# romi/plant-3d-vision

Measured on AMD Instinct MI355X. Metric: Mvoxels*views/sec space-carve, 512^3 x 72 views per MI355X, higher is better.
Workload: dtype f32

## Files before the change

plant-3d-vision_amd/csrc/sc_bricks.h:

```cpp

template <bool ALL_SAFE = false>
__device__ __forceinline__ void two_views(const ViewDesc &da, const ViewDesc &db, bool two, float x, float y,
                                          const float (&z)[4], unsigned long long (&alive)[4], unsigned long long (&kept)[4]) {
    const float aax = da.R[0] * x + da.R[1] * y, aay = da.R[3] * x + da.R[4] * y, aaz = da.R[6] * x + da.R[7] * y;
    const float bax = db.R[0] * x + db.R[1] * y, bay = db.R[3] * x + db.R[4] * y, baz = db.R[6] * x + db.R[7] * y;
    const uint32_t rowa = (uint32_t)da.strip, rowb = (uint32_t)db.strip;
    unsigned long long oka[4], okb[4];
    uint32_t wa[4], wb[4];
    int sha[4], shb[4];
#pragma unroll
    for (int e = 0; e < 4; ++e) {
        int v;
        bool ok = project<ALL_SAFE>(aax, aay, aaz, z[e], da, sha[e], v, oka[e]);
        wa[e] = load_mask_at(da.mask, ok ? mask_byte_offset(sha[e], v, rowa) : 0u);
        ok = project<ALL_SAFE>(bax, bay, baz, z[e], db, shb[e], v, okb[e]);
        wb[e] = load_mask_at(db.mask, ok ? mask_byte_offset(shb[e], v, rowb) : 0u);
    }
    const unsigned long long second = two ? ~0ull : 0ull;
#pragma unroll
    for (int e = 0; e < 4; ++e) {
        unsigned long long fg = __ballot(__builtin_amdgcn_ubfe(wa[e], (uint32_t)sha[e], 1u) != 0u);
        unsigned long long seen = oka[e] & alive[e];
        alive[e] &= ~(seen & ~fg);
        kept[e] |= seen & fg;
        fg = __ballot(__builtin_amdgcn_ubfe(wb[e], (uint32_t)shb[e], 1u) != 0u);
        seen = okb[e] & alive[e] & second;
        alive[e] &= ~(seen & ~fg);
        kept[e] |= seen & fg;
    }
}

__device__ __forceinline__ void labels_behind(int32_t (&lab)[4], const unsigned long long (&alive)[4],
                                              const unsigned long long (&kept)[4]) {
#pragma unroll
    for (int e = 0; e < 4; ++e) {
        const int32_t up = lab[e] == 0 ? 1 : lab[e];
        const int32_t live = __builtin_amdgcn_inverse_ballot_w64(kept[e]) ? up : lab[e];
        lab[e] = __builtin_amdgcn_inverse_ballot_w64(alive[e]) ? live : -1;
    }
}

template <bool FRESH, bool ALL_SAFE = false>
__device__ __forceinline__ void brick_voxels(int32_t *__restrict__ labels, const GridDesc &g,
                                             const ViewDesc *__restrict__ views, int nviews,
                                             int32_t init, Append ap, uint32_t il, uint32_t j,
                                             uint32_t k0, uint32_t lb, uint32_t lane, uint32_t unit = 0,
                                             int nextra = 0) {
    const bool inside = j < g.ny && k0 < g.nz;
    const int nvalid = inside ? (int)min(4u, g.nz - k0) : 0;
    const uint64_t elem = ((uint64_t)il * g.ny + j) * g.nzp + k0;
    int32_t *p = labels + elem;
    int32_t lab[4], was[4];
#pragma unroll
    for (int e = 0; e < 4; ++e) lab[e] = -1;
    if (FRESH) {
#pragma unroll
        for (int e = 0; e < 4; ++e)
            if (e < nvalid) lab[e] = init;
    } else if (inside) {
        int4 q = *reinterpret_cast<const int4 *>(p);
        lab[0] = q.x; lab[1] = q.y; lab[2] = q.z; lab[3] = q.w;
#pragma unroll
        for (int e = 0; e < 4; ++e)
            if (e >= nvalid) lab[e] = -1;
    }
    unsigned long long alive[4], kept[4];
#pragma unroll
    for (int e = 0; e < 4; ++e) {
        was[e] = lab[e];
        alive[e] = __ballot(lab[e] != -1);
        kept[e] = 0;
    }
    const float x = g.ox + (float)(int)(il * g.istride + g.i0) * g.vs;
    const float y = g.oy + (float)(int)j * g.vs;
    float z[4];
#pragma unroll
    for (int e = 0; e < 4; ++e) z[e] = g.oz + (float)(int)(k0 + e) * g.vs;

    for (int vi = 0; vi < nviews; vi += 2) {
        if ((alive[0] | alive[1] | alive[2] | alive[3]) == 0) break;
        const bool two = vi + 1 < nviews;
        const ViewDesc da = views[vi];
        const ViewDesc db = views[two ? vi + 1 : vi];
        two_views<ALL_SAFE>(da, db, two, x, y, z, alive, kept);
    }
    if (nextra >= 2 && ap.list != nullptr) {
        const uint32_t left = (uint32_t)(__popcll(alive[0]) + __popcll(alive[1]) + __popcll(alive[2]) + __popcll(alive[3]));
        if (left >= 32u && left <= 128u) {
            const ViewDesc da = views[nviews];
            const ViewDesc db = views[nviews + 1];
            two_views<ALL_SAFE>(da, db, true, x, y, z, alive, kept);
        }
    }
    labels_behind(lab, alive, kept);

    const bool changed = FRESH || lab[0] != was[0] || lab[1] != was[1] || lab[2] != was[2] || lab[3] != was[3];
    if (inside && changed) *reinterpret_cast<int4 *>(p) = make_int4(lab[0], lab[1], lab[2], lab[3]);

    if (ap.list != nullptr) {
        ap.sub = (lb * 0x9E3779B1u) >> 24;
        uint32_t total = 0;
#pragma unroll
        for (int e = 0; e < 4; ++e) total += (uint32_t)__popcll(alive[e]);
        bool bulked = false;
        if (ap.bulk != nullptr && total >= ap.bulk_min) {
            uint32_t pos = 0;
            if (lane == 0) pos = atomicAdd(&ap.ctl->count[3][ap.sub].n, 1u);
            pos = __shfl(pos, 0);
            bulked = pos < ap.bulkcap;
            if (bulked && lane == 0)
                ap.bulk[(size_t)ap.sub * ap.bulkcap + pos] = lb * 4u + unit;
        }
        if (total != 0 && !bulked) {
            uint32_t base = 0;
            if (lane == 0) base = atomicAdd(&ap.ctl->count[0][ap.sub].n, total);
            base = __shfl(base, 0);
            if (base + total > ap.subcap) {
                if (lane == 0) ap.ctl->overflow = 1u;
            } else {
                uint32_t *dst = ap.list + (size_t)ap.sub * ap.subcap + base;
                uint32_t rank = 0;
#pragma unroll
                for (int e = 0; e < 4; ++e) rank += lanes_below(alive[e]);
#pragma unroll
                for (int e = 0; e < 4; ++e) {
                    if (__builtin_amdgcn_inverse_ballot_w64(alive[e])) {
                        dst[rank] = (uint32_t)(elem + e) | (lab[e] == 0 ? 0x80000000u : 0u);
                        ++rank;
                    }
                }
            }
        }
    }
}

struct Fill {
    int32_t kept;
    int32_t fresh;
    int32_t init;
};

__device__ __forceinline__ uint32_t strip_flag(const uint8_t *__restrict__ flags, uint32_t strip, uint32_t bricks_z) {
    const uint32_t lane = threadIdx.x & 63;
    return (lane < bricks_z) ? flags[strip * bricks_z + lane] : 0u;
}
__device__ __forceinline__ void store_culled_bricks(int32_t *__restrict__ labels, const GridDesc &g, uint32_t f, uint32_t strip,
                                                    uint32_t bricks_y, uint32_t bricks_z, Fill fill, bool prefilled = false) {
    typedef int v4i __attribute__((ext_vector_type(4)));
    const uint32_t wave = __builtin_amdgcn_readfirstlane(threadIdx.x >> 6), lane = threadIdx.x & 63;
    const uint32_t il = strip / bricks_y, by = strip - il * bricks_y;
    const uint32_t j0 = by * kBrickY + wave * 4, j = j0 + (lane >> 4);
    const unsigned long long culled = prefilled ? 0ull : __ballot(f == 1u), full = __ballot(f == 2u);
    const unsigned long long untouched = fill.fresh ? __ballot(f == 6u) : 0ull;
    if (j >= g.ny) return;
    const uint32_t l16 = lane & 15u;
    const bool tail_ok = (bricks_z - 1u) * kBrickZ + l16 * 4u < g.nz;
    const unsigned long long last = 1ull << (bricks_z - 1u);
    {
        const char *wbase = reinterpret_cast<const char *>(labels) + ((uint64_t)il * g.ny + j0) * g.nzp * 4u;
        const uint32_t voff = (lane >> 4) * g.nzp * 4u + l16 * 16u;
        v4i minus = {-1, -1, -1, -1};
        asm volatile("" : "+v"(minus));
        unsigned long long body = culled & ~last;
        while (body != 0) {
            const uint32_t bz = (uint32_t)__builtin_ctzll(body);
            body &= body - 1;
            asm volatile("global_store_dwordx4 %0, %1, %2 nt" ::"v"(voff), "v"(minus), "s"(wbase + bz * 256u) : "memory");
        }
        if ((culled & last) != 0 && tail_ok)
            asm volatile("global_store_dwordx4 %0, %1, %2 nt" ::"v"(voff), "v"(minus), "s"(wbase + (bricks_z - 1u) * 256u) : "memory");
        asm volatile("s_nop 1" ::"v"(minus));
    }
    unsigned long long rest = full | untouched;
    if (rest == 0) return;
    int32_t *col = labels + ((uint64_t)il * g.ny + j) * g.nzp;
    while (rest != 0) {
        const uint32_t bz = (uint32_t)__builtin_ctzll(rest);
        rest &= rest - 1;
        const bool isfull = (full >> bz) & 1ull;
        const uint32_t k0 = bz * kBrickZ + l16 * 4;
        if (k0 >= g.nz) continue;
        if (!isfull || fill.fresh) {
            const int32_t val = isfull ? fill.kept : fill.init;
            const v4i vv = {val, val, val, val};
            __builtin_nontemporal_store(vv, reinterpret_cast<v4i *>(col + k0));
        } else {
            const uint32_t n = min(4u, g.nz - k0);
            for (uint32_t e = 0; e < n; ++e)
                if (col[k0 + e] == 0) col[k0 + e] = 1;
        }
    }
}

#ifdef SC_TRACE_DENSE
__device__ uint32_t g_dense_trace[8192 * 8];
#endif
constexpr int kConfirmWaves = 8;
struct UnitRoad {
    int32_t *labels;
    int32_t init, fresh;
    uint32_t nbricks;
};

__global__ __launch_bounds__(64 * kConfirmWaves) void brick_confirm_kernel(
    GridDesc g, const ViewDesc *__restrict__ views, int v0, int v1, uint32_t bricks_y, uint32_t bricks_z,
    uint8_t *__restrict__ flags, const uint32_t *__restrict__ cands, uint32_t cand_per, uint32_t *__restrict__ late,
    ListCtl *ctl, uint32_t parity, UnitRoad ur) {
    if (v0 >= v1) return;
    uint32_t ncand[kCandSub], gfirst[kCandSub + 1];
    gfirst[0] = 0;
#pragma unroll
    for (int s = 0; s < kCandSub; ++s) {
        ncand[s] = ctl->ncand[parity][s].n;
        gfirst[s + 1] = gfirst[s] + ((ncand[s] + 63u) >> 6);
    }
    __shared__ unsigned long long s_full[kConfirmWaves], s_seen[kConfirmWaves];
    __shared__ unsigned long long s_road, s_rseen;
    const uint32_t wave = __builtin_amdgcn_readfirstlane(threadIdx.x >> 6), lane = threadIdx.x & 63u;
    const uint32_t per_plane = bricks_y * bricks_z;
    for (uint32_t grp = blockIdx.x; grp < gfirst[kCandSub]; grp += gridDim.x) {
        uint32_t sub = 0, first = 0, n = ncand[0];
#pragma unroll
        for (int s = 1; s < kCandSub; ++s)
            if (grp >= gfirst[s]) { sub = (uint32_t)s; first = gfirst[s]; n = ncand[s]; }
        const uint32_t idx = (grp - first) * 64u + lane;
        const bool isc = idx < n;
        const uint32_t lb = isc ? cands[(size_t)sub * cand_per * 64u + idx] : 0u;
        const uint32_t fl = isc ? flags[lb] : 0u;
        unsigned long long any_seen = __ballot(fl == 3u);
        unsigned long long cand = __ballot(isc);
        const uint32_t il = lb / per_plane;
        const uint32_t rem = lb - il * per_plane;
        const uint32_t by = rem / bricks_z, bz = rem - by * bricks_z;
        const float x = g.ox + (float)(int)(il * g.istride + g.i0) * g.vs;
        for (int base = v0; base < v1 && cand != 0; base += kConfirmWaves) {
            const int vi = base + (int)wave;
            bool keeps = true, sees = false;
            if (vi < v1 && ((cand >> lane) & 1ull)) {
                const ViewDesc d = views[vi];
                const uint32_t v = brick_verdict(d, g, x, (int)(by * kBrickY), (int)(bz * kBrickZ), d.tiles_x);
                keeps = v == 2u || v == 4u;
                sees = v == 2u;
            }
            const unsigned long long mf = __ballot(keeps), ms = __ballot(sees);
            __syncthreads();
            if (lane == 0) { s_full[wave] = mf; s_seen[wave] = ms; }
            __syncthreads();
#pragma unroll
            for (int w = 0; w < kConfirmWaves; ++w) { cand &= s_full[w]; any_seen |= s_seen[w]; }
        }
        const bool road = ur.labels != nullptr && ctl->overflow == 0u;
        if (wave == 0) {
            if (isc) flags[lb] = ((cand >> lane) & 1ull) ? (((any_seen >> lane) & 1ull) ? 2 : 6) : 5;
            const bool failed = isc && !((cand >> lane) & 1ull);
            const unsigned long long m = __ballot(failed);
            if (m != 0) {
                uint32_t pos = 0;
                if (lane == 0) pos = atomicAdd(road ? &ctl->nlate_units : &ctl->nlate, (uint32_t)__popcll(m));
                pos = __shfl(pos, 0);
                const unsigned long long below = (lane == 0) ? 0ull : (~0ull >> (64 - lane));
                const uint32_t at = pos + (uint32_t)__popcll(m & below);
                if (failed) late[road ? ur.nbricks - 1u - at : at] = lb;
            }
            if (lane == 0) { s_road = road ? m : 0ull; s_rseen = any_seen; }
        }
        __syncthreads();
        if (road) {
            const unsigned long long mr = s_road, ms = s_rseen;
            uint32_t nth = 0;
            for (unsigned long long mm = mr; mm != 0; mm &= mm - 1, ++nth) {
                if ((nth & (uint32_t)(kConfirmWaves - 1)) != wave) continue;
                const uint32_t src = (uint32_t)__builtin_ctzll(mm);
                const uint32_t b = __builtin_amdgcn_readlane(lb, src);
                const bool seen = (ms >> src) & 1ull;
                const uint32_t bil = b / per_plane, brem = b - bil * per_plane;
                const uint32_t bby = brem / bricks_z, bbz = brem - bby * bricks_z;
                const uint32_t k0 = bbz * kBrickZ + (lane & 15u) * 4u;
#pragma unroll
                for (uint32_t i = 0; i < 4u; ++i) {
                    const uint32_t j = bby * kBrickY + i * 4u + (lane >> 4);
                    if (j >= g.ny || k0 >= g.nz) continue;
                    int32_t *p = ur.labels + ((uint64_t)bil * g.ny + j) * g.nzp + k0;
                    if (ur.fresh) {
                        const int32_t val = (seen && ur.init == 0) ? 1 : ur.init;
                        *reinterpret_cast<int4 *>(p) = make_int4(val, val, val, val);
                    } else if (seen) {
                        int4 q = *reinterpret_cast<const int4 *>(p);
                        const bool changed = q.x == 0 || q.y == 0 || q.z == 0 || q.w == 0;
                        q.x = q.x == 0 ? 1 : q.x; q.y = q.y == 0 ? 1 : q.y; q.z = q.z == 0 ? 1 : q.z; q.w = q.w == 0 ? 1 : q.w;
                        if (changed) *reinterpret_cast<int4 *>(p) = q;
                    }
                }
            }
        }
        __syncthreads();
    }
}

template <bool FRESH, bool ALL_SAFE = false>
__global__ __launch_bounds__(kBlock) __attribute__((amdgpu_num_sgpr(102))) void carve_brick_kernel(int32_t *__restrict__ labels, GridDesc g,
                                                             const ViewDesc *__restrict__ views,
                                                             int nviews, int32_t init, Append ap,
                                                             uint32_t bricks_y, uint32_t bricks_z,
                                                             const uint8_t *__restrict__ flags,
                                                             const uint32_t *__restrict__ live,
                                                             ListCtl *ctl, uint32_t nwalkers,
                                                             PackJob ride, int pack_rows,
                                                             uint32_t parity, int nverd_arg, uint32_t verd_max_live,
                                                             uint32_t bulk_min_live, int nextra) {
    if (blockIdx.x >= nwalkers) {
        const uint32_t b = blockIdx.x - nwalkers;
        const int rs = pack_rows == 0 ? pack_band_slot(ride, b)
                                      : (pack_rows == 1 ? pack16_slot<1>(ride, b)
                                                        : (pack_rows == 2 ? pack16_slot<2>(ride, b) : (pack_rows == 8 ? pack16_slot<8>(ride, b) : pack16_slot<4>(ride, b))));
        if (rs >= ride.nslots) return;
        const TileRect rc = job_rect(ride, rs + ride.slot0);
        uint32_t packed;
        if (pack_rows == 0) packed = pack_band_block(ride, b, rc);
        else if (pack_rows == 1) packed = pack16_block<1>(ride, b, rc);
        else if (pack_rows == 2) packed = pack16_block<2>(ride, b, rc);
        else if (pack_rows == 8) packed = pack16_block<8>(ride, b, rc);
        else packed = pack16_block<4>(ride, b, rc);
        if (packed != 0u && threadIdx.x == 0) (void)atomicAdd(&ctl->rider_tiles[b & (uint32_t)(kRiderCounters - 1)].n, packed);
        return;
    }
    const uint32_t nlive = ctl->nlive[parity];
    const int nverd = nlive <= verd_max_live ? nverd_arg : 0;
    if (nlive < bulk_min_live) ap.bulk = nullptr;
    const uint32_t lane = threadIdx.x & 63;
    const uint32_t per_plane = bricks_y * bricks_z;
    const uint32_t xcd = blockIdx.x & 7u;
    const uint32_t per_xcd = (nwalkers >> 3) * (kBlock / 64);
    bool first = true;
    uint32_t misses = 0, turn = 0;
#ifdef SC_TRACE_DENSE
    const uint64_t tr0 = wall_clock64();
    uint32_t tr_bricks = 0, tr_units = 0, tr_verd = 0, tr_unit = 0, tr_tick = 0;
#endif
    for (;;) {
#ifdef SC_TRACE_DENSE
        const uint64_t tra = wall_clock64();
// ... 158 lines not shown
```

plant-3d-vision_amd/csrc/sc_engine.h:

```cpp

struct sc_engine {
    int device = 0;
    int mode = SC_MODE_CARVE;
    int64_t nx = 0, ny = 0, nz = 0, i0 = 0, istride = 1, planes = 0, n = 0;
    int64_t nzp = 0;
    int64_t npitch = 0;
    void *dense = nullptr;
    float origin[3] = {0, 0, 0};
    float vs = 1.0f;
    float default_value = 0.0f;
    void *state = nullptr;
    bool fresh = true;

    hipStream_t own_stream = nullptr, stream = nullptr;
    std::thread setup_thread;
    bool setup_pending = false;
    int setup_rc = SC_OK;
    std::string setup_err;
    double setup_ms = 0.0;
    double setup_waited_ms = 0.0;

    std::vector<ViewDesc> pending;
    ViewDesc *views_dev = nullptr;
    ViewDesc *views_pin = nullptr;
// ... 473 lines not shown
    for (int q = 0; q < V; ++q) {
        ViewDesc d;
        fill_desc(e, d, K + 4 * q, R + 9 * q, t + 3 * q,
                  static_cast<uint32_t *>(packed) + (size_t)q * words, H, W, occ + (size_t)q * occ_bytes);
        if (cmask) d.cmask = cmask + (size_t)q * occ_bytes;
        e->pending.push_back(d);
    }
    return SC_OK;
}

int enqueue_tile8(sc_engine *e, int V, const float *K, const float *R, const float *t,
                  const void *raw_dev, int H, int W, int64_t row_stride, int64_t view_stride) {
    int tiles_x = (W + kATileW - 1) / kATileW, tiles_y = (H + kATileH - 1) / kATileH;
    size_t per_view = (size_t)tiles_x * tiles_y * 128;
    if (per_view >= ((size_t)1 << 31) || (size_t)tiles_y * 128 >= ((size_t)1 << 24))
        return fail(SC_ERR_INVALID, "mask too large for the byte gather (%d x %d)", W, H);
    void *tiled = nullptr;
    int rc = arena_alloc(e, per_view * (size_t)V, &tiled);
    if (rc) return rc;
    int fast = (W % 16) == 0 && (row_stride % 16) == 0 && (view_stride % 16) == 0 &&
               (reinterpret_cast<uintptr_t>(raw_dev) % 16) == 0;
    int64_t total = (int64_t)V * H * ((W + 15) / 16);
    int64_t blocks = (total + kBlock - 1) / kBlock;
    if (blocks > 0x7fffffffLL) return fail(SC_ERR_INVALID, "mask batch too large");
    const size_t uni_per_view = (size_t)((W + 31) / 32) * (size_t)((H + 31) / 32);
    uint8_t *uni = nullptr;
    if (fast && e->avg_brick) {
        void *u = nullptr;
        size_t bytes = (uni_per_view * (size_t)V + 3) & ~(size_t)3;
        rc = arena_alloc(e, bytes, &u);
        if (rc) return rc;
        uni = static_cast<uint8_t *>(u);
    }
    LaunchTimer lt{e, SC_KERNEL_PACK};
    rc = lt.begin();
    if (rc) return rc;
    hipLaunchKernelGGL(tile8_kernel, dim3((uint32_t)blocks), dim3(kBlock), 0, e->stream,
                       static_cast<const uint8_t *>(raw_dev), row_stride, view_stride, W, H, V, tiles_x,
                       tiles_y, static_cast<uint8_t *>(tiled), fast);
    if (uni) {
        int64_t ntiles = (int64_t)V * (int64_t)uni_per_view;
        hipLaunchKernelGGL(uniform_tiles_kernel, dim3((uint32_t)((ntiles + 3) / 4)), dim3(kBlock), 0, e->stream,
                           static_cast<const uint8_t *>(tiled), W, H, V, tiles_x, tiles_y, uni);
    }
    HIP_TRY(hipGetLastError());
    rc = lt.end();
    if (rc) return rc;
    for (int q = 0; q < V; ++q) {
        ViewDesc d;
        fill_desc(e, d, K + 4 * q, R + 9 * q, t + 3 * q, static_cast<uint8_t *>(tiled) + (size_t)q * per_view, H, W,
                  uni ? uni + (size_t)q * uni_per_view : nullptr);
        d.tiles_x = tiles_y * 128;
        d.pad = 1;
        e->pending.push_back(d);
    }
    return SC_OK;
}

int enqueue_tilef32(sc_engine *e, int V, const float *K, const float *R, const float *t, const void *raw_dev,
                    int H, int W, int64_t row_stride, int64_t view_stride) {
    const int tiles_x = (W + kFTileW - 1) / kFTileW, tiles_y = (H + kFTileH - 1) / kFTileH;
    const size_t per_view = (size_t)tiles_x * tiles_y * 128;
    if (per_view >= ((size_t)1 << 33) || (size_t)tiles_y * 32 >= ((size_t)1 << 24))
        return fail(SC_ERR_INVALID, "mask too large for the float gather (%d x %d)", W, H);
    void *tiled = nullptr;
    int rc = arena_alloc(e, per_view * (size_t)V, &tiled);
    if (rc) return rc;
    const int fast = (W % 4) == 0 && (row_stride % 16) == 0 && (view_stride % 16) == 0 &&
                     (reinterpret_cast<uintptr_t>(raw_dev) % 16) == 0;
    const int64_t total = (int64_t)V * H * ((W + 3) / 4);
    const int64_t blocks = (total + kBlock - 1) / kBlock;
    if (blocks > 0x7fffffffLL) return fail(SC_ERR_INVALID, "mask batch too large");
    const size_t nreg = (size_t)((W + 31) / 32) * (size_t)((H + 31) / 32);
    const size_t uni_view = ((nreg + 3) & ~(size_t)3) + nreg * 4;
    void *u = nullptr;
    rc = arena_alloc(e, uni_view * (size_t)V, &u);
    if (rc) return rc;
    uint8_t *uni = static_cast<uint8_t *>(u);
    LaunchTimer lt{e, SC_KERNEL_PACK};
    rc = lt.begin();
    if (rc) return rc;
    hipLaunchKernelGGL(tilef_kernel, dim3((uint32_t)blocks), dim3(kBlock), 0, e->stream, static_cast<const float *>(raw_dev),
                       row_stride, view_stride, W, H, V, tiles_x, tiles_y, static_cast<float *>(tiled), fast);
    const int64_t regs = (int64_t)V * (int64_t)nreg;
    hipLaunchKernelGGL(uniform_f32_kernel, dim3((uint32_t)((regs + 3) / 4)), dim3(kBlock), 0, e->stream,
                       static_cast<const float *>(tiled), W, H, V, tiles_x, tiles_y, uni, uni_view);
    HIP_TRY(hipGetLastError());
    rc = lt.end();
    if (rc) return rc;
    for (int q = 0; q < V; ++q) {
        ViewDesc d;
        fill_desc(e, d, K + 4 * q, R + 9 * q, t + 3 * q, static_cast<char *>(tiled) + (size_t)q * per_view, H, W,
                  uni + (size_t)q * uni_view);
        d.tiles_x = tiles_y * 32;
        d.pad = 2;
        e->pending.push_back(d);
    }
    return SC_OK;
}

void order_views(std::vector<ViewDesc> &v, std::vector<uint32_t> *perm = nullptr) {
    size_t n = v.size();
    if (perm) {
        perm->resize(n);
        for (size_t q = 0; q < n; ++q) (*perm)[q] = (uint32_t)q;
    }
    if (n < 3 || n > 4096) return;
    std::vector<float> worst(n, 0.0f);
    std::vector<char> used(n, 0);
    std::vector<ViewDesc> out;
    out.reserve(n);
    size_t cur = 0;
    for (size_t step = 0; step < n; ++step) {
        used[cur] = 1;
        out.push_back(v[cur]);
        if (perm) (*perm)[step] = (uint32_t)cur;
        const float *a = v[cur].R + 6;
        size_t best = n;
        for (size_t q = 0; q < n; ++q) {
            if (used[q]) continue;
            const float *b = v[q].R + 6;
            float c = std::fabs(a[0] * b[0] + a[1] * b[1] + a[2] * b[2]);
            if (c > worst[q]) worst[q] = c;
            if (best == n || worst[q] < worst[best]) best = q;
        }
        cur = best;
    }
    v.swap(out);
}

constexpr int kMinFusedViews = 6;

int ensure_lists(sc_engine *e) {
    if (e->lists && e->list_cap_built == e->list_cap) return SC_OK;
    if (e->lists) {
        HIP_TRY(schost::wait_stream(e->stream));
        (void)hipFree(e->lists);
        e->lists = nullptr;
    }
    uint64_t total = std::max<uint64_t>((uint64_t)e->n / 4 + (uint64_t)e->n / 16, (uint64_t)kSub * 1024);
    e->subcap = (uint32_t)((total + kSub - 1) / kSub);
    if (e->list_cap > 0) e->subcap = (uint32_t)e->list_cap;
    HIP_TRY(sc_dev_malloc(reinterpret_cast<void **>(&e->lists), (size_t)2 * kSub * e->subcap * sizeof(uint32_t)));
    e->list_cap_built = e->list_cap;
    return SC_OK;
}

int ensure_ctl(sc_engine *e) {
    if (e->ctl) return SC_OK;
    size_t nbricks = 0;
    if ((e->nz + kBrickZ - 1) / kBrickZ <= 64)
        nbricks = (size_t)e->planes * (size_t)((e->ny + kBrickY - 1) / kBrickY) * (size_t)((e->nz + kBrickZ - 1) / kBrickZ);
    char *base = nullptr;
    size_t flag_bytes = (nbricks + 15) & ~(size_t)15;
    const uint32_t bulkcap = (uint32_t)((nbricks * 4 * 2 + kSub - 1) / kSub + 64);
    const size_t bulk_words = nbricks ? (size_t)kSub * bulkcap : 0;
    const uint32_t itemcap = bulkcap * 5u;
    uint4 *items = nullptr;
    if (bulk_words) HIP_TRY(sc_dev_malloc(reinterpret_cast<void **>(&items), (size_t)kSub * itemcap * sizeof(uint4)));
    hipError_t he = sc_dev_malloc(reinterpret_cast<void **>(&base),
                              2 * sizeof(ListCtl) + flag_bytes + (3 * nbricks + bulk_words) * sizeof(uint32_t) + 16);
    if (he == hipSuccess) he = hipMemsetAsync(base, 0, 2 * sizeof(ListCtl), e->stream);
    if (he != hipSuccess) {
        if (items) (void)hipFree(items);
        if (base) (void)hipFree(base);
        return fail(he == hipErrorOutOfMemory ? SC_ERR_NOMEM : SC_ERR_DEVICE, "control block allocation failed: %s", hipGetErrorString(he));
    }
    e->bulkcap = bulkcap;
    e->itemcap = itemcap;
    e->items = items;
    e->ctl2[0] = reinterpret_cast<ListCtl *>(base);
    e->ctl2[1] = e->ctl2[0] + 1;
    e->ctl_clean[0] = e->ctl_clean[1] = true;
    e->ctl_idx = 0;
    e->ctl = e->ctl2[0];
    e->flags = reinterpret_cast<uint8_t *>(base + 2 * sizeof(ListCtl));
    e->live = reinterpret_cast<uint32_t *>(base + 2 * sizeof(ListCtl) + flag_bytes);
    e->late = e->live + nbricks;
    e->fill_list = e->late + nbricks;
    e->bulk = bulk_words ? e->fill_list + nbricks : nullptr;
    return SC_OK;
}

int deferred_job(sc_engine *e, PackJob *out) {
    const auto &db = e->deferred;
    size_t words = packed_words(db.H, db.W);
    void *packed = nullptr, *occ_v = nullptr;
    int rc = arena_alloc(e, words * 4 * (size_t)db.V, &packed);
    if (rc) return rc;
    const size_t occ_bytes = (size_t)((db.W + kTile - 1) / kTile) * (size_t)((db.H + kTile - 1) / kTile);
    rc = arena_alloc(e, occ_bytes * (size_t)db.V, &occ_v);
    if (rc) return rc;
    uint32_t *cmask = nullptr;
    if (e->bulk_min > 0 || e->unit_cull) {
        void *cv = nullptr;
        rc = arena_alloc(e, occ_bytes * 4 * (size_t)db.V, &cv);
        if (rc) return rc;
        cmask = static_cast<uint32_t *>(cv);
    }
    for (int q = 0; q < db.V; ++q) {
        e->pending[(size_t)q].mask = static_cast<uint32_t *>(packed) + (size_t)q * words;
        e->pending[(size_t)q].occ = static_cast<uint8_t *>(occ_v) + (size_t)q * occ_bytes;
        if (cmask) e->pending[(size_t)q].cmask = cmask + (size_t)q * occ_bytes;
    }
    *out = make_pack_job(db.raw, db.row_stride, db.view_stride, db.W, db.H, static_cast<uint32_t *>(packed),
                         (int64_t)words, pack_flip(db.dtype), static_cast<uint8_t *>(occ_v), cmask);
    return SC_OK;
}

int materialize_deferred(sc_engine *e) {
    if (!e->deferred.on) return SC_OK;
    PackJob pj;
    int rc = deferred_job(e, &pj);
    if (rc) return rc;
    e->deferred.on = false;
    pj.slot0 = 0;
    pj.nslots = e->deferred.V;
    rc = step_begin(e);
    if (rc) return rc;
    LaunchTimer lt{e, SC_KERNEL_PACK};
    rc = lt.begin();
    if (rc) return rc;
    rc = launch_pack16(e, pj);
    if (rc) return rc;
    return lt.end();
}

int hostbits_reserve(sc_engine *e, size_t bytes, char **out) {
    auto &a = e->hb[e->hb_cur];
    if (a.used == 0 && a.armed) {
        HIP_TRY(schost::wait_event(a.ev));
        a.armed = false;
    }
    if (a.used + bytes > a.cap) {
        const size_t cap = std::max<size_t>({a.used + bytes, a.cap * 2, (size_t)16 << 20});
        char *pin = nullptr, *dev = nullptr;
        HIP_TRY(sc_pin_malloc(reinterpret_cast<void **>(&pin), cap, hipHostMallocDefault));
        hipError_t he = sc_dev_malloc(reinterpret_cast<void **>(&dev), cap);
        if (he != hipSuccess) {
            (void)hipHostFree(pin);
            return fail(he == hipErrorOutOfMemory ? SC_ERR_NOMEM : SC_ERR_DEVICE, "host-mask arena: %s", hipGetErrorString(he));
        }
        if (a.used) memcpy(pin, a.pin, a.used);
        if (a.pin) {
            HIP_TRY(schost::wait_stream(e->stream));
            (void)hipHostFree(a.pin);
            (void)hipFree(a.dev);
        }
        a.pin = pin;
        a.dev = dev;
        a.cap = cap;
        a.armed = false;
    }
    if (!a.ev) HIP_TRY(hipEventCreateWithFlags(&a.ev, hipEventDisableTiming));
    *out = a.pin + a.used;
    a.used += bytes;
    return SC_OK;
}

int hostbits_push_view(sc_engine *e, const float *K, const float *R, const float *t, uint64_t src_off, int H, int W);

int enqueue_hostbits(sc_engine *e, const float *K, const float *R, const float *t, const void *mask, int H, int W,
                     int dtype, int64_t row_stride) {
    const int wpr = (W + kTile - 1) / kTile;
    const size_t bits_bytes = ((size_t)H * wpr * 4 + 255) & ~(size_t)255;
    char *dst = nullptr;
    int rc = hostbits_reserve(e, bits_bytes, &dst);
    if (rc) return rc;
    const uint64_t src_off = (uint64_t)(dst - e->hb[e->hb_cur].pin);
    const int elem = dtype == SC_MASK_I32 ? 4 : 1;
    const uint8_t flip = dtype == SC_MASK_U8_INV ? 255 : dtype == SC_MASK_BOOL_INV ? 1 : 0;
    uint32_t *out = reinterpret_cast<uint32_t *>(dst);
    const bool par = (size_t)H * W >= ((size_t)1 << 18);
    const int band = 64, nparts = par ? (H + band - 1) / band : 1;
    schost::parallel_for(nparts, [&](int part) {
        const int r0 = par ? part * band : 0, r1 = par ? std::min(H, r0 + band) : H;
        schost::pack_rows(mask, row_stride, W, r0, r1, out, wpr, elem, flip);
    });
    return hostbits_push_view(e, K, R, t, src_off, H, W);
}

int hostbits_push_view(sc_engine *e, const float *K, const float *R, const float *t, uint64_t src_off, int H, int W) {
    const int wpr = (W + kTile - 1) / kTile, tiles_y = (H + kTile - 1) / kTile;
    const size_t ntiles = (size_t)wpr * tiles_y;
    void *tiles = nullptr, *occ = nullptr, *cm = nullptr;
    int rc = arena_alloc(e, ntiles * 128, &tiles);
    if (rc) return rc;
    rc = arena_alloc(e, ntiles, &occ);
    if (rc) return rc;
    rc = arena_alloc(e, ntiles * 4, &cm);
    if (rc) return rc;
    BitsRec br;
    memset(&br, 0, sizeof br);
    br.src_off = src_off;
    br.tiles = static_cast<uint32_t *>(tiles);
    br.occ = static_cast<uint8_t *>(occ);
    br.cmask = static_cast<uint32_t *>(cm);
    br.W = W; br.H = H; br.tiles_x = wpr; br.tiles_y = tiles_y;
    e->hp_pending.push_back(br);
    ViewDesc d;
    fill_desc(e, d, K, R, t, tiles, H, W, static_cast<const uint8_t *>(occ));
    d.cmask = static_cast<const uint32_t *>(cm);
    e->pending.push_back(d);
    return SC_OK;
}

int upload_hostbits(sc_engine *e) {
// ... 32 lines not shown
```

plant-3d-vision_amd/csrc/sc_lists.h:

```cpp

struct UnitItems {
    const uint4 *items;
    uint32_t cap;
    const ViewDesc *views;
    uint32_t bricks_y, bricks_z;
};

__device__ __forceinline__ uint32_t list_reserve(ListCounter *counter, uint32_t total, uint32_t cap, uint32_t lane) {
    uint32_t base = 0;
    if (lane == 0) {
        base = atomicAdd(&counter->n, total);
        if (base > cap || total > cap - base) {
            atomicMax(&counter->cut, ~min(base, cap));
            base = 0xffffffffu;
        }
    }
    return __shfl(base, 0);
}

struct UnitSpill {
    const uint32_t *units;
    uint32_t cap, floor;
    uint32_t bricks_y, bricks_z;
};

template <bool FINAL, int P, bool ALL_SAFE = false>
__global__ __launch_bounds__(kBlock) __attribute__((amdgpu_num_sgpr(96))) void carve_list_kernel(int32_t *__restrict__ labels, GridDesc g,
                                                            const ViewDesc *__restrict__ views,
                                                            int nviews,
                                                            const uint32_t *__restrict__ lin,
                                                            uint32_t *__restrict__ lout,
                                                            ListCtl *ctl, int sin, int sout,
                                                            uint32_t subcap, int vgsize, CullStores cs, UnitItems ui,
                                                            UnitSpill us, int nrest) {
    static_assert(P == 2, "two survivors per lane: the instances with one and with four were retired in round 6");
    __shared__ uint32_t pref[kSub + 1];
    const uint32_t tid = threadIdx.x;
    const uint32_t bx = blockIdx.x, gdim = gridDim.x;
    const bool split = cs.flags != nullptr;
    const uint32_t nown = cs.nstrips - cs.first, nvirt = nown + cs.spec;
    const uint32_t nstore = split ? (cs.fill_blocks ? cs.fill_blocks : nvirt) : 0u;
    const uint32_t nbid = gdim - nstore;
    if (split && bx >= nbid) {
        constexpr uint32_t kAhead = 4;
        for (uint32_t t = bx - nbid; t < nvirt; t += nstore * kAhead) {
            uint32_t f[kAhead];
#pragma unroll
            for (uint32_t u = 0; u < kAhead; ++u) {
                const uint32_t tt = t + u * nstore;
                f[u] = tt < nvirt ? strip_flag(cs.flags, tt < nown ? cs.first + tt : tt - nown, cs.bricks_z) : 0u;
            }
#pragma unroll
            for (uint32_t u = 0; u < kAhead; ++u) {
                const uint32_t tt = t + u * nstore;
                if (tt < nvirt)
                    store_culled_bricks(labels, g, f[u], tt < nown ? cs.first + tt : tt - nown, cs.bricks_y, cs.bricks_z,
                                        Fill{cs.kept, cs.fresh, cs.init}, tt >= nown);
            }
        }
        return;
    }
    if (ctl->overflow) return;
    const uint32_t bid = bx;
    constexpr uint32_t CH = 64u * P;
    {
        uint32_t c = (list_count(ctl->count[sin][tid], subcap) + CH - 1u) / CH;
        if (tid == 0) pref[0] = 0;
        pref[tid + 1] = c;
        __syncthreads();
        for (uint32_t off = 1; off < kSub; off <<= 1) {
            uint32_t val = pref[tid + 1];
            uint32_t add = (tid >= off) ? pref[tid + 1 - off] : 0u;
            __syncthreads();
            pref[tid + 1] = val + add;
            __syncthreads();
        }
    }
    const uint32_t chunks = pref[kSub];
    const uint32_t lane = tid & 63u;
    __shared__ uint32_t ipref[kSub + 1];
    const bool with_items = FINAL && ui.items != nullptr;
    uint32_t uchunks = 0;
    constexpr uint32_t kUnitParts = 256u / (64u * P);
    if (!FINAL && us.units != nullptr) {
        const uint32_t c = min(ctl->count[3][tid].n, us.cap);
        if (tid == 0) ipref[0] = 0;
        ipref[tid + 1] = c;
        __syncthreads();
        for (uint32_t off = 1; off < kSub; off <<= 1) {
            const uint32_t val = ipref[tid + 1];
            const uint32_t add = (tid >= off) ? ipref[tid + 1 - off] : 0u;
            __syncthreads();
            ipref[tid + 1] = val + add;
            __syncthreads();
        }
        if (ipref[kSub] < us.floor) uchunks = ipref[kSub] * kUnitParts;
    }
    if (with_items) {
        const uint32_t c = list_count(ctl->count[4][tid], ui.cap);
        if (tid == 0) ipref[0] = 0;
        ipref[tid + 1] = c;
        __syncthreads();
        for (uint32_t off = 1; off < kSub; off <<= 1) {
            const uint32_t val = ipref[tid + 1];
            const uint32_t add = (tid >= off) ? ipref[tid + 1 - off] : 0u;
            __syncthreads();
            ipref[tid + 1] = val + add;
            __syncthreads();
        }
    }
    const uint64_t nworkers = (uint64_t)nbid * (kBlock / 64);
    const uint32_t wave = __builtin_amdgcn_readfirstlane(tid >> 6);
    const uint64_t total = FINAL ? (uint64_t)chunks * (uint32_t)nviews : (uint64_t)chunks + uchunks;
    uint64_t per = 1;
    if (FINAL) {
        per = (total + nworkers - 1) / nworkers;
        const uint64_t r = (uint64_t)max(vgsize, 1);
        per = (per + r - 1) / r * r;
    }
    const uint64_t wid = (uint64_t)bid * (kBlock / 64) + wave;
    uint64_t pos = FINAL ? min(total, wid * per) : wid;
    const uint64_t end = FINAL ? min(total, pos + per) : total;
    while (pos < end) {
        uint32_t c;
        int v0, v1;
        if (FINAL) {
            c = (uint32_t)(pos / (uint32_t)nviews);
            v0 = (int)(pos - (uint64_t)c * (uint32_t)nviews);
            v1 = (int)min((uint64_t)nviews, (uint64_t)v0 + (end - pos));
            pos += (uint64_t)(v1 - v0);
        } else {
            c = (uint32_t)pos;
            v0 = 0;
            v1 = nviews;
            pos += nworkers;
        }
        const bool from_unit = !FINAL && c >= chunks;
        const uint32_t *pf = from_unit ? ipref : pref;
        const uint32_t key = from_unit ? (c - chunks) / kUnitParts : c;
        uint32_t lo = 0, hi = kSub;
        while (hi - lo > 1) {
            uint32_t mid = (lo + hi) >> 1;
            if (pf[mid] <= key) lo = mid; else hi = mid;
        }
        const uint32_t s = lo;
        const uint32_t cnt = list_count(ctl->count[sin][s], subcap);
        uint32_t idx[P];
        unsigned long long alive_m[P], zero_m[P], flip_m[P];
        float x[P], y[P], z[P];
        uint32_t unit = 0, upart = 0;
        if (from_unit) {
            unit = __builtin_amdgcn_readfirstlane(us.units[(size_t)s * us.cap + (key - ipref[s])]);
            upart = (c - chunks) % kUnitParts;
        }
#pragma unroll
        for (int p = 0; p < P; ++p) {
            if (from_unit) {
                const uint32_t v = upart * CH + (uint32_t)p * 64u + lane;
                const uint32_t lb = unit >> 2, per_plane = us.bricks_y * us.bricks_z;
                const uint32_t il = lb / per_plane, rem = lb - il * per_plane;
                const uint32_t by = rem / us.bricks_z, bz = rem - by * us.bricks_z;
                const uint32_t j = by * kBrickY + (v >> 4), k = bz * kBrickZ + (unit & 3u) * 16u + (v & 15u);
                const bool inside = j < g.ny && k < g.nz;
                idx[p] = inside ? (il * g.ny + j) * g.nzp + k : 0u;
                int32_t lab = -1;
                if (inside) lab = labels[idx[p]];
                alive_m[p] = __ballot(lab != -1);
                zero_m[p] = __ballot(lab == 0);
            } else {
                const uint32_t e = (c - pref[s]) * CH + (uint32_t)p * 64u + lane;
                const bool in = e < cnt;
                uint32_t entry = 0;
                if (in) entry = lin[(size_t)s * subcap + e];
                idx[p] = entry & 0x7fffffffu;
                alive_m[p] = __ballot(in);
                zero_m[p] = __ballot((entry >> 31) != 0);
            }
            flip_m[p] = 0;
            const uint32_t col = fdiv(idx[p], g.by_nzp);
            const uint32_t k = idx[p] - col * g.nzp;
            const uint32_t il = fdiv(col, g.by_ny);
            const uint32_t j = col - il * g.ny;
            x[p] = g.ox + (float)(int)(il * g.istride + g.i0) * g.vs;
            y[p] = g.oy + (float)(int)j * g.vs;
            z[p] = g.oz + (float)(int)k * g.vs;
        }
        constexpr int U = 4;
        for (;;) {
        for (int vi = v0; vi < v1; vi += U) {
            unsigned long long any = 0;
#pragma unroll
            for (int p = 0; p < P; ++p) any |= alive_m[p];
            if (any == 0) break;
            unsigned long long okm[U][P];
            uint32_t w[U][P];
            int sh[U][P];
#pragma unroll
            for (int q = 0; q < U; ++q) {
                const ViewDesc d = views[vi + q < v1 ? vi + q : vi];
                asm volatile("" ::"s"(d.Wf), "s"(d.Hf), "s"(d.strip), "s"(d.mask));
                const uint32_t tile_row = (uint32_t)d.strip;
#pragma unroll
                for (int p = 0; p < P; ++p) {
                    int vv;
                    const bool ok = project<ALL_SAFE>(d.R[0] * x[p] + d.R[1] * y[p], d.R[3] * x[p] + d.R[4] * y[p],
                                                      d.R[6] * x[p] + d.R[7] * y[p], z[p], d, sh[q][p], vv, okm[q][p]);
                    w[q][p] = 0;
                    if (ok) w[q][p] = load_mask_at(d.mask, mask_byte_offset(sh[q][p], vv, tile_row));
                }
            }
#pragma unroll
// ... 484 lines not shown
```

Before: 68.02 million.

## Read brick flags as scalar words and batch culled-brick stores per strip piece

The store-only blocks of the carve kernel now load each strip's brick flags as three uniform dwords through the constant address space, replacing one per-lane byte load followed by ballots. Flags are decoded eight bricks at a time with SWAR byte compares. A fully culled 8-brick piece takes a fast path that issues eight back-to-back nontemporal stores with immediate offsets. Flag loads are software-pipelined one batch ahead, and the flag buffer gains 12 bytes of padding so the over-read stays in bounds. The cost is more scalar registers and more complex indexing, and the split into 8-brick pieces adds loop iterations when bricks_z is large.

Measured after the change: 65.21 million. -4.1%, worse.

```diff
diff --git a/plant-3d-vision_amd/csrc/sc_bricks.h b/plant-3d-vision_amd/csrc/sc_bricks.h
--- a/plant-3d-vision_amd/csrc/sc_bricks.h
+++ b/plant-3d-vision_amd/csrc/sc_bricks.h
@@ -140,53 +140,100 @@
     int32_t init;
 };
 
-__device__ __forceinline__ uint32_t strip_flag(const uint8_t *__restrict__ flags, uint32_t strip, uint32_t bricks_z) {
-    const uint32_t lane = threadIdx.x & 63;
-    return (lane < bricks_z) ? flags[strip * bricks_z + lane] : 0u;
-}
-__device__ __forceinline__ void store_culled_bricks(int32_t *__restrict__ labels, const GridDesc &g, uint32_t f, uint32_t strip,
-                                                    uint32_t bricks_y, uint32_t bricks_z, Fill fill, bool prefilled = false) {
+struct StripRaw {
+    uint32_t w[3];
+};
+__device__ __forceinline__ StripRaw strip_words_ask(const uint8_t *flags, uint32_t byte0) {
+    StripRaw r{{0u, 0u, 0u}};
+#if defined(__HIP_DEVICE_COMPILE__)
+    typedef const __attribute__((address_space(4))) uint32_t *const_words_t;
+    const const_words_t p = (const_words_t)((uintptr_t)flags + (__builtin_amdgcn_readfirstlane(byte0) & ~3u));
+    r.w[0] = p[0];
+    r.w[1] = p[1];
+    r.w[2] = p[2];
+#endif
+    return r;
+}
+__device__ __forceinline__ unsigned long long strip_words(const StripRaw &r, uint32_t byte0, uint32_t n) {
+    const uint32_t sh = (byte0 & 3u) * 8u;
+    const uint32_t lo = (uint32_t)((((unsigned long long)r.w[1] << 32) | r.w[0]) >> sh);
+    const uint32_t hi = (uint32_t)((((unsigned long long)r.w[2] << 32) | r.w[1]) >> sh);
+    const unsigned long long valid = n >= 8u ? ~0ull : (1ull << (8u * n)) - 1ull;
+    return (((unsigned long long)hi << 32) | lo) & valid;
+}
+__device__ __forceinline__ unsigned long long bytes_equal(unsigned long long w, uint32_t code) {
+    constexpr unsigned long long k7f = 0x7f7f7f7f7f7f7f7full;
+    const unsigned long long x = w ^ (0x0101010101010101ull * code);
+    return ~(((x & k7f) + k7f) | x | k7f);
+}
+
+__device__ __forceinline__ void store_culled_bricks(int32_t *__restrict__ labels, const char *vol, const GridDesc &g, unsigned long long w,
+                                                    uint32_t strip, uint32_t bz0, uint32_t n, uint32_t bricks_y,
+                                                    uint32_t bricks_z, Fill fill, bool prefilled,
+                                                    uint32_t voff, const int __attribute__((ext_vector_type(4))) &minus) {
     typedef int v4i __attribute__((ext_vector_type(4)));
+    const unsigned long long full = bytes_equal(w, 2u);
+    const unsigned long long untouched = fill.fresh ? bytes_equal(w, 6u) : 0ull;
+    const unsigned long long rest0 = full | untouched;
+    if (prefilled && rest0 == 0) return;
     const uint32_t wave = __builtin_amdgcn_readfirstlane(threadIdx.x >> 6), lane = threadIdx.x & 63;
     const uint32_t il = strip / bricks_y, by = strip - il * bricks_y;
     const uint32_t j0 = by * kBrickY + wave * 4, j = j0 + (lane >> 4);
-    const unsigned long long culled = prefilled ? 0ull : __ballot(f == 1u), full = __ballot(f == 2u);
-    const unsigned long long untouched = fill.fresh ? __ballot(f == 6u) : 0ull;
-    if (j >= g.ny) return;
     const uint32_t l16 = lane & 15u;
+    const bool mine = j < g.ny;
     const bool tail_ok = (bricks_z - 1u) * kBrickZ + l16 * 4u < g.nz;
-    const unsigned long long last = 1ull << (bricks_z - 1u);
-    {
-        const char *wbase = reinterpret_cast<const char *>(labels) + ((uint64_t)il * g.ny + j0) * g.nzp * 4u;
-        const uint32_t voff = (lane >> 4) * g.nzp * 4u + l16 * 16u;
-        v4i minus = {-1, -1, -1, -1};
-        asm volatile("" : "+v"(minus));
-        unsigned long long body = culled & ~last;
-        while (body != 0) {
-            const uint32_t bz = (uint32_t)__builtin_ctzll(body);
-            body &= body - 1;
-            asm volatile("global_store_dwordx4 %0, %1, %2 nt" ::"v"(voff), "v"(minus), "s"(wbase + bz * 256u) : "memory");
-        }
-        if ((culled & last) != 0 && tail_ok)
-            asm volatile("global_store_dwordx4 %0, %1, %2 nt" ::"v"(voff), "v"(minus), "s"(wbase + (bricks_z - 1u) * 256u) : "memory");
+    const bool has_last = bz0 + n == bricks_z;
+    const char *wbase = vol + (((uint64_t)il * g.ny + j0) * g.nzp + bz0 * kBrickZ) * 4u;
+    if (!prefilled && mine) {
+        const unsigned long long all = 0x0101010101010101ull >> (8u * (8u - n));
+        if (w == all) {
+            const bool whole = !has_last || (bricks_z - 1u) * kBrickZ + 60u < g.nz;
+            const uint32_t body = whole ? n : n - 1u;
+            if (body == 8u) {
+                asm volatile("global_store_dwordx4 %0, %1, %2 nt\n\t"
+                             "global_store_dwordx4 %0, %1, %2 offset:256 nt\n\t"
+                             "global_store_dwordx4 %0, %1, %2 offset:512 nt\n\t"
+                             "global_store_dwordx4 %0, %1, %2 offset:768 nt\n\t"
+                             "global_store_dwordx4 %0, %1, %2 offset:1024 nt\n\t"
+                             "global_store_dwordx4 %0, %1, %2 offset:1280 nt\n\t"
+                             "global_store_dwordx4 %0, %1, %2 offset:1536 nt\n\t"
+                             "global_store_dwordx4 %0, %1, %2 offset:1792 nt" ::"v"(voff), "v"(minus), "s"(wbase) : "memory");
+            } else {
+                for (uint32_t b = 0; b < body; ++b)
+                    asm volatile("global_store_dwordx4 %0, %1, %2 nt" ::"v"(voff), "v"(minus), "s"(wbase + b * 256u) : "memory");
+                if (!whole && tail_ok)
+                    asm volatile("global_store_dwordx4 %0, %1, %2 nt" ::"v"(voff), "v"(minus), "s"(wbase + (n - 1u) * 256u) : "memory");
+            }
+        } else {
+            const unsigned long long culled = bytes_equal(w, 1u);
+            const unsigned long long last = has_last ? 0x80ull << (8u * (n - 1u)) : 0ull;
+            unsigned long long body = culled & ~last;
+            while (body != 0) {
+                const uint32_t b8 = (uint32_t)__builtin_ctzll(body) & ~7u;
+                body &= body - 1;
+                asm volatile("global_store_dwordx4 %0, %1, %2 nt" ::"v"(voff), "v"(minus), "s"(wbase + b8 * 32u) : "memory");
+            }
+            if ((culled & last) != 0 && tail_ok)
+                asm volatile("global_store_dwordx4 %0, %1, %2 nt" ::"v"(voff), "v"(minus), "s"(wbase + (n - 1u) * 256u) : "memory");
+        }
         asm volatile("s_nop 1" ::"v"(minus));
     }
-    unsigned long long rest = full | untouched;
-    if (rest == 0) return;
+    unsigned long long rest = rest0;
+    if (rest == 0 || !mine) return;
     int32_t *col = labels + ((uint64_t)il * g.ny + j) * g.nzp;
     while (rest != 0) {
-        const uint32_t bz = (uint32_t)__builtin_ctzll(rest);
+        const uint32_t bit = (uint32_t)__builtin_ctzll(rest);
         rest &= rest - 1;
-        const bool isfull = (full >> bz) & 1ull;
-        const uint32_t k0 = bz * kBrickZ + l16 * 4;
+        const bool isfull = (full >> bit) & 1ull;
+        const uint32_t k0 = (bz0 + (bit >> 3)) * kBrickZ + l16 * 4;
         if (k0 >= g.nz) continue;
         if (!isfull || fill.fresh) {
             const int32_t val = isfull ? fill.kept : fill.init;
             const v4i vv = {val, val, val, val};
             __builtin_nontemporal_store(vv, reinterpret_cast<v4i *>(col + k0));
         } else {
-            const uint32_t n = min(4u, g.nz - k0);
-            for (uint32_t e = 0; e < n; ++e)
+            const uint32_t n4 = min(4u, g.nz - k0);
+            for (uint32_t e = 0; e < n4; ++e)
                 if (col[k0 + e] == 0) col[k0 + e] = 1;
         }
     }
diff --git a/plant-3d-vision_amd/csrc/sc_engine.h b/plant-3d-vision_amd/csrc/sc_engine.h
--- a/plant-3d-vision_amd/csrc/sc_engine.h
+++ b/plant-3d-vision_amd/csrc/sc_engine.h
@@ -649,7 +649,7 @@
     if ((e->nz + kBrickZ - 1) / kBrickZ <= 64)
         nbricks = (size_t)e->planes * (size_t)((e->ny + kBrickY - 1) / kBrickY) * (size_t)((e->nz + kBrickZ - 1) / kBrickZ);
     char *base = nullptr;
-    size_t flag_bytes = (nbricks + 15) & ~(size_t)15;
+    size_t flag_bytes = (nbricks + 12 + 15) & ~(size_t)15;
     const uint32_t bulkcap = (uint32_t)((nbricks * 4 * 2 + kSub - 1) / kSub + 64);
     const size_t bulk_words = nbricks ? (size_t)kSub * bulkcap : 0;
     const uint32_t itemcap = bulkcap * 5u;
diff --git a/plant-3d-vision_amd/csrc/sc_lists.h b/plant-3d-vision_amd/csrc/sc_lists.h
--- a/plant-3d-vision_amd/csrc/sc_lists.h
+++ b/plant-3d-vision_amd/csrc/sc_lists.h
@@ -42,21 +42,59 @@
     const uint32_t nstore = split ? (cs.fill_blocks ? cs.fill_blocks : nvirt) : 0u;
     const uint32_t nbid = gdim - nstore;
     if (split && bx >= nbid) {
+        typedef int v4i __attribute__((ext_vector_type(4)));
         constexpr uint32_t kAhead = 4;
-        for (uint32_t t = bx - nbid; t < nvirt; t += nstore * kAhead) {
-            uint32_t f[kAhead];
+        const uint32_t npieces = (cs.bricks_z + 7u) >> 3;
+        const uint32_t l = tid & 63u;
+        const uint32_t voff = (l >> 4) * g.nzp * 4u + (l & 15u) * 16u;
+        v4i minus = {-1, -1, -1, -1};
+        asm volatile("" : "+v"(minus));
+        const char *vol = reinterpret_cast<const char *>(labels);
+        asm volatile("" : "+s"(vol));
+        auto strip_of = [&](uint32_t t) { return t < nown ? cs.first + t : t - nown; };
+        auto byte_of = [&](uint32_t t, uint32_t c) { return strip_of(min(t, nvirt - 1u)) * cs.bricks_z + c * 8u; };
+        auto step = [&](uint32_t &t, uint32_t &c) {
+            const bool wrap = c + 1u == npieces;
+            t = wrap ? t + nstore : t;
+            c = wrap ? 0u : c + 1u;
+        };
+        uint32_t t = bx - nbid, c = 0;
+        StripRaw cur[kAhead];
+        {
+            uint32_t ta = t, ca = c;
 #pragma unroll
             for (uint32_t u = 0; u < kAhead; ++u) {
-                const uint32_t tt = t + u * nstore;
-                f[u] = tt < nvirt ? strip_flag(cs.flags, tt < nown ? cs.first + tt : tt - nown, cs.bricks_z) : 0u;
-            }
+                cur[u] = strip_words_ask(cs.flags, byte_of(ta, ca));
+                step(ta, ca);
+            }
+        }
+        while (t < nvirt) {
+            uint32_t tn = t, cn = c;
+#pragma unroll
+            for (uint32_t u = 0; u < kAhead; ++u) step(tn, cn);
+            StripRaw nxt[kAhead];
+            {
+                uint32_t ta = tn, ca = cn;
+#pragma unroll
+                for (uint32_t u = 0; u < kAhead; ++u) {
+                    nxt[u] = strip_words_ask(cs.flags, byte_of(ta, ca));
+                    step(ta, ca);
+                }
+            }
+            uint32_t ts = t, cq = c;
 #pragma unroll
             for (uint32_t u = 0; u < kAhead; ++u) {
-                const uint32_t tt = t + u * nstore;
-                if (tt < nvirt)
-                    store_culled_bricks(labels, g, f[u], tt < nown ? cs.first + tt : tt - nown, cs.bricks_y, cs.bricks_z,
-                                        Fill{cs.kept, cs.fresh, cs.init}, tt >= nown);
-            }
+                if (ts < nvirt) {
+                    const uint32_t n = min(8u, cs.bricks_z - cq * 8u);
+                    store_culled_bricks(labels, vol, g, strip_words(cur[u], byte_of(ts, cq), n), strip_of(ts), cq * 8u, n, cs.bricks_y,
+                                        cs.bricks_z, Fill{cs.kept, cs.fresh, cs.init}, ts >= nown, voff, minus);
+                }
+                step(ts, cq);
+            }
+#pragma unroll
+            for (uint32_t u = 0; u < kAhead; ++u) cur[u] = nxt[u];
+            t = tn;
+            c = cn;
         }
         return;
     }
```
